# saurabh260918/Graph-Attention-Network-GATv2-

Hardware: AMD Instinct MI355X
Metric: edges/sec (fwd+bwd, 2-layer 8-head GATv2) (higher is better)
Workload: dtype f32; 1 GPU; products-shape synthetic power-law graph, 2450000 nodes / 61900000 edges / 100 feat / 47 classes, 2-layer GATv2 heads [8, 8] outdims [8, 8], fp32; launch=eager, parallelism=single GPU, generator=device (csrc/gat_synth.hip), bit-for-bit synth.py

## Files before the change

graph-attention-network-gatv2-_amd/csrc/gat_dense_kernels.hip:

```cpp
#include "gat_internal.h"

#include <algorithm>
#include <type_traits>

#include <cstdlib>

namespace gat {
namespace {

struct MapIdentity {
    __device__ __forceinline__ int64_t operator()(int64_t idx) const { return idx; }
};
struct MapGradW {
    int32_t HD, F, c_base;
    __device__ __forceinline__ int64_t operator()(int64_t idx) const {
        const int32_t c = c_base + (int32_t)idx / F, f = (int32_t)idx % F;
        return (int64_t)(c % HD) * 2 * F + (c / HD) * F + f;
    }
};
template <class MAP>
__global__ __launch_bounds__(1024) void reduce_slabs_kernel(const float* __restrict__ slabs, int32_t nslabs,
                                                           int64_t width, float* __restrict__ out, MAP map) {
    __shared__ float part[16][64];
    const int q = threadIdx.x & 63, sl = threadIdx.x >> 6;
    const int64_t idx = (int64_t)blockIdx.x * 64 + q;
    float s0 = 0.f, s1 = 0.f, s2 = 0.f, s3 = 0.f;
    if (idx < width) {
        int z = sl;
        for (; z + 48 < nslabs; z += 64) {
            s0 += slabs[(int64_t)z * width + idx];
            s1 += slabs[(int64_t)(z + 16) * width + idx];
            s2 += slabs[(int64_t)(z + 32) * width + idx];
            s3 += slabs[(int64_t)(z + 48) * width + idx];
        }
        for (; z < nslabs; z += 16) s0 += slabs[(int64_t)z * width + idx];
    }
    part[sl][q] = (s0 + s1) + (s2 + s3);
    __syncthreads();
    if (sl == 0 && idx < width) {
        float tot = 0.f;
#pragma unroll
        for (int w = 0; w < 16; ++w) tot += part[w][q];
        out[map(idx)] += tot;
    }
}

__global__ __launch_bounds__(1024) void reduce_batch_kernel(ReduceBatch B) {
    __shared__ float part[16][64];
    if ((int)blockIdx.x >= B.blocks) {
        if (threadIdx.x >= 64) return;
        float lossv = 0.f; int32_t corrv = 0;
        if (B.fin_loss != nullptr) {
            double l = 0.0; int c = 0;
            for (int i = threadIdx.x; i < B.fin_n; i += 64) { l += B.fin_loss[i]; c += B.fin_corr[i]; }
            for (int off = 32; off > 0; off >>= 1) { l += __shfl_down(l, off); c += __shfl_down(c, off); }
            lossv = (float)l; corrv = c;
            if (threadIdx.x == 0) { *B.fin_loss_out = lossv; *B.fin_corr_out = corrv; }
        } else if (threadIdx.x == 0 && B.dst3 != nullptr) {
            lossv = *B.loss; corrv = *B.correct;
        }
        if (threadIdx.x == 0 && B.dst3 != nullptr) {
            const float v0 = lossv, v1 = (float)(corrv & 4095), v2 = (float)(corrv >> 12);
            B.dst3[0] = v0; B.dst3[1] = v1; B.dst3[2] = v2;
            if (B.dst3_host != nullptr) { B.dst3_host[0] = v0; B.dst3_host[1] = v1; B.dst3_host[2] = v2; }
        }
        return;
    }
    int j = 0;
#pragma unroll
    for (int i = 1; i < 8; ++i) if (i < B.n && (int)blockIdx.x >= B.jobs[i].block0) j = i;
    const ReduceJob J = B.jobs[j];
    const int q = threadIdx.x & 63, sl = threadIdx.x >> 6;
    const int64_t idx = (int64_t)((int)blockIdx.x - J.block0) * 64 + q;
    float s0 = 0.f, s1 = 0.f, s2 = 0.f, s3 = 0.f;
    if (idx < J.width) {
        int z = sl;
        for (; z + 48 < J.nslabs; z += 64) {
            s0 += J.slabs[(int64_t)z * J.width + idx];
            s1 += J.slabs[(int64_t)(z + 16) * J.width + idx];
            s2 += J.slabs[(int64_t)(z + 32) * J.width + idx];
            s3 += J.slabs[(int64_t)(z + 48) * J.width + idx];
        }
        for (; z < J.nslabs; z += 16) s0 += J.slabs[(int64_t)z * J.width + idx];
    }
    part[sl][q] = (s0 + s1) + (s2 + s3);
    __syncthreads();
    if (sl == 0 && idx < J.width) {
        float tot = 0.f;
#pragma unroll
        for (int w = 0; w < 16; ++w) tot += part[w][q];
        const int64_t o = J.HD != 0 ? MapGradW{J.HD, J.F, J.c_base}(idx) : idx;
        J.out[o] += tot;
    }
}

template <int DLP>
__global__ __launch_bounds__(256) void head_forward_kernel(HeadArgs A, int32_t NB, int32_t ldz) {
    extern __shared__ float lds[];
    constexpr int DLS = DLP > 0 ? DLP : 1;
    const int C = A.C, DL = A.DL;
    const int wstride = DLP > 0 ? DLP : DL;
    float* s_wo = lds;
    float* s_z = lds + C * wstride;
    __shared__ double s_loss[4];
    __shared__ int32_t s_corr[4];
    for (int i = threadIdx.x; i < C * wstride; i += blockDim.x) {
        const int c = i / wstride, j = i % wstride;
        s_wo[i] = j < DL ? A.Wo[c * DL + j] : 0.f;
    }
    __syncthreads();
    double loss_acc = 0.0;
    int corr_acc = 0;
    const int64_t ntiles = (A.n_rows + NB - 1) / NB;
    const int dq = 256 / C, dr = 256 % C;
    for (int64_t tile = blockIdx.x; tile < ntiles; tile += gridDim.x) {
        const int64_t n0 = tile * NB;
        const int t = threadIdx.x;
        const int64_t n = n0 + t;
        if (t < NB && n < A.n_rows) {
            float* zr = s_z + t * ldz;
            const float* x = A.HL + n * DL;
            float mv = -INFINITY;
            if constexpr (DLP > 0) {
                float xr[DLS];
#pragma unroll
                for (int j = 0; j < DLS; ++j) xr[j] = j < DL ? x[j] : 0.f;
                for (int c = 0; c < C; ++c) {
                    float acc = 0.f;
#pragma unroll
                    for (int j = 0; j < DLS; ++j) acc += s_wo[c * DLS + j] * xr[j];
                    zr[c] = acc;
                    mv = fmaxf(mv, acc);
                }
            } else {
                for (int c = 0; c < C; ++c) {
                    float acc = 0.f;
                    for (int j = 0; j < DL; ++j) acc += s_wo[c * DL + j] * x[j];
                    zr[c] = acc;
                    mv = fmaxf(mv, acc);
                }
            }
            float sum = 0.f;
            for (int c = 0; c < C; ++c) { const float ev = __builtin_amdgcn_exp2f((zr[c] - mv) * 1.4426950408889634f); zr[c] = ev; sum += ev; }
            const double den = (double)sum + 1e-8;
            const double rden = 1.0 / den;
            const int lab = A.labels[n];
            float best = -1.f; int pred = 0; float plab = 0.f;
            for (int c = 0; c < C; ++c) {
                const float yv = (float)((double)zr[c] * rden);
                zr[c] = yv;
                if (c == 0 || yv > best) { best = yv; pred = c; }
                if (c == lab) plab = yv;
            }
            loss_acc += lab >= 0 ? (double)(-logf(fmaxf(plab, 1e-12f))) : 0.0;
            corr_acc += (lab >= 0 && pred == lab) ? 1 : 0;
// ... 126 lines not shown
    const int tid = threadIdx.x;
    const int t2 = tid - 128;
    const int wc = t2 >= 0 ? t2 % C : 0, whalf = t2 >= 0 ? t2 / C : 2;
    float wacc[DL];
#pragma unroll
    for (int d = 0; d < DL; ++d) wacc[d] = 0.f;
    const int64_t ntiles = (A.n_rows + NB - 1) / NB;
    const int dqC = 256 / C, drC = 256 % C;
    for (int64_t tile = blockIdx.x; tile < ntiles; tile += gridDim.x) {
        const int64_t n0 = tile * NB;
        const int rows_here = (int)((A.n_rows - n0 < NB) ? (A.n_rows - n0) : NB);
        __syncthreads();
        {
            const float* yt = A.y + n0 * C;
            int r = tid / C, c = tid % C;
            for (int q = tid; q < rows_here * C; q += 256) {
                const int lab_r = A.labels[n0 + r];
                s_dz[r * ldz + c] = lab_r >= 0 ? yt[q] - (c == lab_r ? 1.0f : 0.0f) : 0.0f;
                r += dqC; c += drC;
                if (c >= C) { c -= C; ++r; }
            }
        }
        for (int q = tid; q < rows_here * DL; q += 256) s_hl[q] = A.HL[n0 * DL + q];
        __syncthreads();
        if (tid < 128) {
            if (tid < rows_here) {
                float acc[DL];
#pragma unroll
                for (int d = 0; d < DL; ++d) acc[d] = 0.f;
                const float* zr = s_dz + tid * ldz;
                for (int c = 0; c < C; ++c) {
                    const float z = zr[c];
#pragma unroll
                    for (int d = 0; d < DL; ++d) acc[d] += s_wo[c * DL + d] * z;
                }
                float* out = A.gh_out + (n0 + tid) * (A.gh_stride ? A.gh_stride : DL);
#pragma unroll
                for (int d = 0; d < DL; ++d) out[d] = acc[d];
            }
        } else if (whalf < 2) {
            const int r0 = whalf * 64, r1 = (r0 + 64 < rows_here) ? r0 + 64 : rows_here;
            for (int r = r0; r < r1; ++r) {
                const float z = s_dz[r * ldz + wc];
#pragma unroll
                for (int d = 0; d < DL; ++d) wacc[d] += z * s_hl[r * DL + d];
            }
        }
    }
    __syncthreads();
    float* s_tmp = s_dz;
    if (whalf < 2) {
#pragma unroll
        for (int d = 0; d < DL; ++d) s_tmp[(whalf * C + wc) * DL + d] = wacc[d];
    }
    __syncthreads();
    for (int i = tid; i < C * DL; i += 256) A.partial[(int64_t)blockIdx.x * C * DL + i] = s_tmp[i] + s_tmp[C * DL + i];
}

template <int DL>
__global__ __launch_bounds__(256) void head_step_kernel(HeadArgs F, HeadBwdArgs A, int32_t ldz) {
    constexpr int NB = 128;
    extern __shared__ float lds[];
    const int C = A.C;
    float* s_wo = lds;
    float* s_dz = s_wo + C * DL;
    float* s_hl = s_dz + NB * ldz;
    __shared__ double s_loss[2];
    __shared__ int32_t s_corr[2];
    for (int i = threadIdx.x; i < C * DL; i += 256) s_wo[i] = A.Wo[i];
    const int tid = threadIdx.x;
    const int t2 = tid - 128;
    const int wc = t2 >= 0 ? t2 % C : 0, whalf = t2 >= 0 ? t2 / C : 2;
    float wacc[DL];
#pragma unroll
    for (int d = 0; d < DL; ++d) wacc[d] = 0.f;
    double loss_acc = 0.0;
    int corr_acc = 0;
    const int64_t ntiles = (A.n_rows + NB - 1) / NB;
    for (int64_t tile = blockIdx.x; tile < ntiles; tile += gridDim.x) {
        const int64_t n0 = tile * NB;
        const int rows_here = (int)((A.n_rows - n0 < NB) ? (A.n_rows - n0) : NB);
        __syncthreads();
        if (tid < rows_here) {
            const int64_t n = n0 + tid;
            float x[DL];
#pragma unroll
            for (int j = 0; j < DL; ++j) { x[j] = A.HL[n * DL + j]; s_hl[tid * DL + j] = x[j]; }
            float* zr = s_dz + tid * ldz;
            float mv = -INFINITY;
            for (int c = 0; c < C; ++c) {
                float acc = 0.f;
#pragma unroll
                for (int j = 0; j < DL; ++j) acc += s_wo[c * DL + j] * x[j];
                zr[c] = acc;
                mv = fmaxf(mv, acc);
            }
            float sum = 0.f;
            for (int c = 0; c < C; ++c) { const float ev = __builtin_amdgcn_exp2f((zr[c] - mv) * 1.4426950408889634f); zr[c] = ev; sum += ev; }
            const double rden = 1.0 / ((double)sum + 1e-8);
            const int lab = A.labels[n];
            float best = -1.f; int pred = 0; float plab = 0.f;
            for (int c = 0; c < C; ++c) {
                const float yv = (float)((double)zr[c] * rden);
                if (c == 0 || yv > best) { best = yv; pred = c; }
                if (c == lab) plab = yv;
                zr[c] = lab >= 0 ? yv - (c == lab ? 1.0f : 0.0f) : 0.0f;
            }
            loss_acc += lab >= 0 ? (double)(-logf(fmaxf(plab, 1e-12f))) : 0.0;
            corr_acc += (lab >= 0 && pred == lab) ? 1 : 0;
        }
        __syncthreads();
        if (tid < 128) {
            if (tid < rows_here) {
                float acc[DL];
#pragma unroll
                for (int d = 0; d < DL; ++d) acc[d] = 0.f;
                const float* zr = s_dz + tid * ldz;
                for (int c = 0; c < C; ++c) {
                    const float z = zr[c];
#pragma unroll
                    for (int d = 0; d < DL; ++d) acc[d] += s_wo[c * DL + d] * z;
                }
                if (A.gh_out != nullptr) {
                    float* out = A.gh_out + (n0 + tid) * (A.gh_stride ? A.gh_stride : DL);
#pragma unroll
                    for (int d = 0; d < DL; ++d) out[d] = acc[d];
                }
            }
        } else if (whalf < 2) {
            const int r0 = whalf * 64, r1 = (r0 + 64 < rows_here) ? r0 + 64 : rows_here;
            for (int r = r0; r < r1; ++r) {
                const float z = s_dz[r * ldz + wc];
#pragma unroll
                for (int d = 0; d < DL; ++d) wacc[d] += z * s_hl[r * DL + d];
            }
        }
    }
    __syncthreads();
    float* s_tmp = s_dz;
    if (whalf < 2) {
#pragma unroll
        for (int d = 0; d < DL; ++d) s_tmp[(whalf * C + wc) * DL + d] = wacc[d];
    }
    for (int off = 32; off > 0; off >>= 1) {
        loss_acc += __shfl_down(loss_acc, off);
        corr_acc += __shfl_down(corr_acc, off);
    }
    if (tid < 128 && (tid & 63) == 0) { s_loss[tid >> 6] = loss_acc; s_corr[tid >> 6] = corr_acc; }
    __syncthreads();
    for (int i = tid; i < C * DL; i += 256) A.partial[(int64_t)blockIdx.x * C * DL + i] = s_tmp[i] + s_tmp[C * DL + i];
    if (tid == 0) {
        F.loss_partial[blockIdx.x] = s_loss[0] + s_loss[1];
        F.correct_partial[blockIdx.x] = s_corr[0] + s_corr[1];
    }
}

__global__ __launch_bounds__(256) void sgd_kernel(float* p, const float* g, float lr, int64_t n) {
    const int64_t i = (int64_t)blockIdx.x * blockDim.x + threadIdx.x;
    if (i < n) p[i] -= lr * g[i];
}
__global__ __launch_bounds__(256) void adam_kernel(float* p, const float* g, float* m, float* v, float lr,
                                                  int64_t n, float b1, float b2, float eps, int32_t t) {
    const int64_t i = (int64_t)blockIdx.x * blockDim.x + threadIdx.x;
    if (i < n) {
        const float gi = g[i];
        const float mi = b1 * m[i] + (1.0f - b1) * gi;
        const float vi = b2 * v[i] + (1.0f - b2) * (gi * gi);
        m[i] = mi; v[i] = vi;
        const float mh = mi / (1.0f - powf(b1, (float)t));
        const float vh = vi / (1.0f - powf(b2, (float)t));
        p[i] -= lr * mh / (sqrtf(vh) + eps);
    }
}
__global__ __launch_bounds__(1024) void sumsq_kernel(const float* __restrict__ g, int64_t n, float* out) {
    __shared__ float part[16];
    float s = 0.f;
    for (int64_t i = threadIdx.x; i < n; i += blockDim.x) s += g[i] * g[i];
    for (int off = 32; off > 0; off >>= 1) s += __shfl_down(s, off);
    if ((threadIdx.x & 63) == 0) part[threadIdx.x >> 6] = s;
    __syncthreads();
    if (threadIdx.x == 0) {
        float t = 0.f;
        for (int w = 0; w < 16; ++w) t += part[w];
        *out = t;
    }
}
__global__ __launch_bounds__(256) void clip_scale_kernel(float* g, int64_t n, const float* sumsq, float thresh) {
    const float norm = sqrtf(*sumsq);
    float scale = 1.0f;
    if (norm > thresh) scale = thresh / (norm + 1e-9f);
    if (!(scale < 1.0f)) return;
    const int64_t i = (int64_t)blockIdx.x * blockDim.x + threadIdx.x;
    if (i < n) g[i] *= scale;
}

template <int V>
__global__ __launch_bounds__(256) void res_backward_kernel(ResBwdArgs A, int32_t LPR, int32_t rpb) {
    __shared__ float red[256 * 4];
    const int HD = A.H * A.D;
    const int t = threadIdx.x;
    const int r_in = t / LPR, cl = t % LPR;
    const float inv_heads = 1.0f / (float)A.H;
    for (int base = 0; base < HD; base += LPR * V) {
        const int c0 = base + cl * V;
        const bool active = r_in < rpb && c0 < HD;
        float sum[V];
        float bv[V];
#pragma unroll
        for (int i = 0; i < V; ++i) { sum[i] = 0.f; bv[i] = (active && A.bias != nullptr) ? A.bias[c0 + i] : 0.f; }
        if (active) {
            for (int64_t row = (int64_t)blockIdx.x * rpb + r_in; row < A.n_rows; row += (int64_t)gridDim.x * rpb) {
                const int64_t o = row * HD + c0;
                float hp[V], gv[V], rv[V];
                if constexpr (V == 4) {
                    const float4 h4 = *reinterpret_cast<const float4*>(A.hpre + o);
                    hp[0] = h4.x; hp[1] = h4.y; hp[2] = h4.z; hp[3] = h4.w;
                    float4 r4 = make_float4(0.f, 0.f, 0.f, 0.f);
                    if (A.res != nullptr) r4 = *reinterpret_cast<const float4*>(A.res + o);
                    rv[0] = r4.x; rv[1] = r4.y; rv[2] = r4.z; rv[3] = r4.w;
                    if (A.gh == nullptr) {
                        const float4 g4 = *reinterpret_cast<const float4*>(A.g + o);
                        gv[0] = g4.x; gv[1] = g4.y; gv[2] = g4.z; gv[3] = g4.w;
                    }
                } else {
                    hp[0] = A.hpre[o];
                    rv[0] = A.res != nullptr ? A.res[o] : 0.f;
                    if (A.gh == nullptr) gv[0] = A.g[o];
                }
                float G[V], ag[V];
#pragma unroll
                for (int i = 0; i < V; ++i) {
                    const float d = hp[i] > 0.f ? 1.0f : A.slope;
                    if (A.gh != nullptr) G[i] = A.gh[row * A.gh_stride + (c0 + i) % A.D] * d * inv_heads;
                    else G[i] = A.g_raw ? gv[i] * d : gv[i];
                    ag[i] = hp[i] - (rv[i] + bv[i]);
                    sum[i] += G[i];
                }
                if constexpr (V == 4) {
                    *reinterpret_cast<float4*>(A.G + o) = make_float4(G[0], G[1], G[2], G[3]);
                    *reinterpret_cast<float4*>(A.agg + o) = make_float4(ag[0], ag[1], ag[2], ag[3]);
                } else {
                    A.G[o] = G[0];
                    A.agg[o] = ag[0];
                }
            }
        }
        if (A.partial != nullptr) {
#pragma unroll
            for (int i = 0; i < V; ++i) red[t * V + i] = sum[i];
            __syncthreads();
            if (r_in == 0 && c0 < HD) {
#pragma unroll
                for (int i = 0; i < V; ++i) {
                    float tot = 0.f;
                    for (int r = 0; r < rpb; ++r) tot += red[(r * LPR + cl) * V + i];
                    A.partial[(int64_t)blockIdx.x * HD + c0 + i] = tot;
                }
            }
            __syncthreads();
        }
    }
}

__device__ __forceinline__ float row_lanes_sum(float x, int LPR) {
    for (int off = LPR >> 1; off > 0; off >>= 1) x += __shfl_xor(x, off);
    return x;
}
template <int V>
__device__ __forceinline__ void load_channels(const float* __restrict__ p, float (&x)[V]) {
    if constexpr (V == 4) {
        const float4 t = *reinterpret_cast<const float4*>(p);
        x[0] = t.x; x[1] = t.y; x[2] = t.z; x[3] = t.w;
    } else {
        x[0] = p[0];
    }
}
template <int V, bool ONE>
__global__ __launch_bounds__(256) void norm_backward_kernel(NormBwdArgs A, int32_t LPR, int32_t rpb) {
    __shared__ float red[256 * 4];
    const ResBwdArgs& R = A.r;
    const int HD = R.H * R.D;
    const int t = threadIdx.x;
    const int r_in = t / LPR, cl = t % LPR;
    const int span = LPR * V;
    const int walk = ONE ? 1 : HD;
    const float inv_heads = 1.0f / (float)R.H, inv_hd = 1.0f / (float)HD;
    auto channels = [&](int64_t row, int c, float mu, float rstd, float (&u)[V], float (&xh)[V], float (&dv)[V], float (&dxh)[V]) {
        load_channels<V>(R.hpre + row * HD + c, u);
        float go[V];
        if (R.gh == nullptr) load_channels<V>(R.g + row * HD + c, go);
#pragma unroll
        for (int i = 0; i < V; ++i) {
            const float gm = A.gamma[c + i];
            xh[i] = (u[i] - mu) * rstd;
            const float v = gm * xh[i] + A.beta[c + i];
            if (R.gh != nullptr) go[i] = R.gh[row * R.gh_stride + (c + i) % R.D] * inv_heads;
            dv[i] = go[i] * (v > 0.f ? 1.0f : R.slope);
            dxh[i] = dv[i] * gm;
        }
    };
    for (int ob = 0; ob < HD; ob += span) {
        const int c0 = ob + cl * V;
        const bool own = c0 < HD;
        float sG[V], sg[V], sb[V], bv[V];
#pragma unroll
        for (int i = 0; i < V; ++i) { sG[i] = 0.f; sg[i] = 0.f; sb[i] = 0.f; bv[i] = (own && R.bias != nullptr) ? R.bias[c0 + i] : 0.f; }
// ... 69 lines not shown
        flush(sg, A.part_gamma);
        flush(sb, A.part_beta);
        flush(sG, R.partial);
    }
}

}

static void res_backward_shape(int32_t HD, int* V, int* LPR, int* rpb) {
    *V = HD % 4 == 0 ? 4 : 1;
    const int groups = HD / *V;
    *LPR = groups < 256 ? groups : 256;
    *rpb = 256 / *LPR;
}
int res_backward_blocks(int64_t n_rows, int32_t HD) {
    int V, LPR, rpb;
    res_backward_shape(HD, &V, &LPR, &rpb);
    const void* fn = V == 4 ? (const void*)res_backward_kernel<4> : (const void*)res_backward_kernel<1>;
    const int64_t want = std::max<int64_t>(1, (n_rows + rpb - 1) / rpb);
    return (int)std::min({want, resident_blocks(fn, 0), (int64_t)kResPartialRows});
}
int launch_res_backward(const ResBwdArgs& a, hipStream_t s) {
    if (a.n_rows <= 0) return 0;
    if (a.blocks < 1 || a.blocks > kResPartialRows) return fail(GAT_E_INVALID, "res_backward: blocks must come from res_backward_blocks()");
    if (a.gh == nullptr && a.g == nullptr) return fail(GAT_E_INVALID, "res_backward: no output gradient");
    int V, LPR, rpb;
    res_backward_shape(a.H * a.D, &V, &LPR, &rpb);
    if (V == 4) hipLaunchKernelGGL(res_backward_kernel<4>, dim3((unsigned)a.blocks), dim3(256), 0, s, a, LPR, rpb);
    else hipLaunchKernelGGL(res_backward_kernel<1>, dim3((unsigned)a.blocks), dim3(256), 0, s, a, LPR, rpb);
    GAT_HIP(hipGetLastError());
    return 0;
}
static void norm_backward_shape(int32_t HD, int* V, int* LPR, int* rpb, bool* one) {
    *V = HD % 4 == 0 ? 4 : 1;
    const int groups = HD / *V;
    int l = 1;
    while (l < groups && l < 64) l <<= 1;
    *LPR = l;
    *rpb = 256 / l;
    *one = groups <= l;
}
static const void* norm_backward_fn(int V, bool one) {
    if (V == 4) return one ? (const void*)norm_backward_kernel<4, true> : (const void*)norm_backward_kernel<4, false>;
    return one ? (const void*)norm_backward_kernel<1, true> : (const void*)norm_backward_kernel<1, false>;
}
int norm_backward_blocks(int64_t n_rows, int32_t HD) {
    int V, LPR, rpb;
    bool one;
    norm_backward_shape(HD, &V, &LPR, &rpb, &one);
    const int64_t want = std::max<int64_t>(1, (n_rows + rpb - 1) / rpb);
    return (int)std::min({want, resident_blocks(norm_backward_fn(V, one), 0), (int64_t)kResPartialRows});
}
int launch_norm_backward(const NormBwdArgs& a, hipStream_t s) {
    if (a.r.n_rows <= 0) return 0;
    if (a.r.blocks < 1 || a.r.blocks > kResPartialRows) return fail(GAT_E_INVALID, "norm_backward: blocks must come from norm_backward_blocks()");
    if (a.r.gh == nullptr && a.r.g == nullptr) return fail(GAT_E_INVALID, "norm_backward: no output gradient");
    if (a.gamma == nullptr || a.beta == nullptr || a.r.G == nullptr || a.r.H < 1 || a.r.D < 1) return fail(GAT_E_INVALID, "norm_backward: null argument");
    int V, LPR, rpb;
    bool one;
    norm_backward_shape(a.r.H * a.r.D, &V, &LPR, &rpb, &one);
    NormBwdArgs arg = a;
    void* args[] = {&arg, &LPR, &rpb};
    GAT_HIP(hipLaunchKernel(norm_backward_fn(V, one), dim3((unsigned)a.r.blocks), dim3(256), args, 0, s));
    return 0;
}
static thread_local ReduceBatch t_batch;
static thread_local bool t_batch_on = false;
void reduce_batch_begin() { t_batch = ReduceBatch{}; t_batch_on = true; }
void reduce_batch_abort() { t_batch_on = false; }
void reduce_batch_pack(const float* loss, const int32_t* correct, float* dst3, float* dst3_host) {
    t_batch.loss = loss; t_batch.correct = correct; t_batch.dst3 = dst3; t_batch.dst3_host = dst3_host;
}
bool reduce_batch_finalize(const double* lp, const int32_t* cp, int32_t nb, float* loss_out, int32_t* correct_out) {
    if (!t_batch_on || t_batch.fin_loss != nullptr) return false;
    t_batch.fin_loss = lp; t_batch.fin_corr = cp; t_batch.fin_n = nb; t_batch.fin_loss_out = loss_out; t_batch.fin_corr_out = correct_out;
    return true;
}
static bool reduce_batch_push(const float* slabs, int32_t nslabs, int64_t width, float* out, int32_t HD, int32_t F, int32_t c_base) {
    if (!t_batch_on || t_batch.n >= 8 || width <= 0) return false;
    ReduceJob& j = t_batch.jobs[t_batch.n++];
    j = ReduceJob{slabs, out, width, nslabs, HD, F, c_base, t_batch.blocks};
    t_batch.blocks += (int32_t)((width + 63) / 64);
    return true;
}
int reduce_batch_flush(hipStream_t s) {
    if (!t_batch_on) return 0;
    t_batch_on = false;
    const int extra = (t_batch.dst3 != nullptr || t_batch.fin_loss != nullptr) ? 1 : 0;
    if (t_batch.blocks + extra == 0) return 0;
    hipLaunchKernelGGL(reduce_batch_kernel, dim3((unsigned)(t_batch.blocks + extra)), dim3(1024), 0, s, t_batch);
    GAT_HIP(hipGetLastError());
    return 0;
}

int launch_reduce_gradw(const float* slabs, int32_t ksplit, int32_t HD, int32_t F, int32_t c_base, int32_t M,
                        float* gradW, hipStream_t s) {
    const int64_t width = (int64_t)M * F;
    if (reduce_batch_push(slabs, ksplit, width, gradW, HD, F, c_base)) return 0;
    hipLaunchKernelGGL((reduce_slabs_kernel<MapGradW>), dim3((unsigned)((width + 63) / 64)), dim3(1024), 0, s, slabs,
                       ksplit, width, gradW, MapGradW{HD, F, c_base});
    GAT_HIP(hipGetLastError());
    return 0;
}

int launch_reduce_partials_add(const float* partial, int32_t nblocks, int64_t width, float* out, hipStream_t s) {
    if (width <= 0) return 0;
    if (reduce_batch_push(partial, nblocks, width, out, 0, 0, 0)) return 0;
    hipLaunchKernelGGL((reduce_slabs_kernel<MapIdentity>), dim3((unsigned)((width + 63) / 64)), dim3(1024), 0, s,
                       partial, nblocks, width, out, MapIdentity{});
    GAT_HIP(hipGetLastError());
    return 0;
}

static int head_tile(int32_t C, int32_t DL, int32_t extra_per_row, int32_t* NB, int32_t* ldz) {
    const int l = (C % 2 == 0) ? C + 1 : C;
    int64_t budget = 60 * 1024 / 4 - (int64_t)C * DL;
    int nb = 256;
    while (nb >= 32 && (int64_t)nb * (l + extra_per_row) > budget) nb >>= 1;
    if (nb < 32) return fail(GAT_E_UNSUPPORTED, "output head: num_classes*D_last too large for the LDS tile");
    *NB = nb; *ldz = l;
    return 0;
}
int head_blocks(int64_t n_rows) {
    static const int per = [] { const char* e = choice_env("GAT_HEAD_NODES"); const int v = e ? atoi(e) : 0; return v == 256 ? 256 : 128; }();
    const int64_t b = (n_rows + per - 1) / per;
    return (int)(b < 1 ? 1 : (b > 2048 ? 2048 : b));
}
int launch_head_forward(const HeadArgs& a, hipStream_t s) {
    int32_t NB, ldz;
    const int dlp = a.DL <= 8 ? 8 : (a.DL <= 16 ? 16 : (a.DL <= 32 ? 32 : (a.DL <= 64 ? 64 : 0)));
    GAT_TRY(head_tile(a.C, dlp ? dlp : a.DL, 0, &NB, &ldz));
    int blocks = head_blocks(a.n_rows);
    const size_t lds = ((size_t)a.C * (dlp ? dlp : a.DL) + (size_t)NB * ldz) * sizeof(float);
    {
        const void* fn = dlp == 8 ? (const void*)head_forward_kernel<8> : dlp == 16 ? (const void*)head_forward_kernel<16>
                       : dlp == 32 ? (const void*)head_forward_kernel<32> : dlp == 64 ? (const void*)head_forward_kernel<64>
                                                                                      : (const void*)head_forward_kernel<0>;
        const int64_t res = resident_blocks(fn, lds);
        if (res < blocks) blocks = (int)res;
    }
    switch (dlp) {
        case 8: hipLaunchKernelGGL(head_forward_kernel<8>, dim3(blocks), dim3(256), lds, s, a, NB, ldz); break;
        case 16: hipLaunchKernelGGL(head_forward_kernel<16>, dim3(blocks), dim3(256), lds, s, a, NB, ldz); break;
        case 32: hipLaunchKernelGGL(head_forward_kernel<32>, dim3(blocks), dim3(256), lds, s, a, NB, ldz); break;
        case 64: hipLaunchKernelGGL(head_forward_kernel<64>, dim3(blocks), dim3(256), lds, s, a, NB, ldz); break;
        default: hipLaunchKernelGGL(head_forward_kernel<0>, dim3(blocks), dim3(256), lds, s, a, NB, ldz); break;
    }
    GAT_HIP(hipGetLastError());
    hipLaunchKernelGGL(head_finalize_kernel, dim3(1), dim3(64), 0, s, a.loss_partial, a.correct_partial, blocks,
                       a.loss_out, a.correct_out);
    GAT_HIP(hipGetLastError());
    return 0;
}
bool head_step_supported(const HeadBwdArgs& b) {
    return b.g == nullptr && b.gh_out != nullptr && b.C <= 64 && (b.DL == 4 || b.DL == 8 || b.DL == 16);
}
int launch_head_step(const HeadArgs& f, const HeadBwdArgs& b, hipStream_t s) {
    HeadBwdArgs probe = b;
    if (probe.gh_out == nullptr) probe.gh_out = reinterpret_cast<float*>(1);
    if (!head_step_supported(probe)) return fail(GAT_E_UNSUPPORTED, "head_step: shape outside the fused kernel");
    const int ldz = (b.C % 2 == 0) ? b.C + 1 : b.C;
    const size_t lds = ((size_t)b.C * b.DL + (size_t)128 * (ldz + b.DL)) * sizeof(float);
    int blocks = std::min(head_blocks(b.n_rows), head_bwd_blocks(b.n_rows, b.C, b.DL));
    const void* fn = b.DL == 4 ? (const void*)head_step_kernel<4> : b.DL == 8 ? (const void*)head_step_kernel<8>
                                                                                : (const void*)head_step_kernel<16>;
    const int64_t res = resident_blocks(fn, lds);
    if (res < blocks) blocks = (int)res;
    if (blocks < 1) blocks = 1;
    if (b.DL == 4) hipLaunchKernelGGL(head_step_kernel<4>, dim3(blocks), dim3(256), lds, s, f, b, ldz);
    else if (b.DL == 8) hipLaunchKernelGGL(head_step_kernel<8>, dim3(blocks), dim3(256), lds, s, f, b, ldz);
    else hipLaunchKernelGGL(head_step_kernel<16>, dim3(blocks), dim3(256), lds, s, f, b, ldz);
    GAT_HIP(hipGetLastError());
    if (!reduce_batch_finalize(f.loss_partial, f.correct_partial, blocks, f.loss_out, f.correct_out)) {
        hipLaunchKernelGGL(head_finalize_kernel, dim3(1), dim3(64), 0, s, f.loss_partial, f.correct_partial, blocks,
                           f.loss_out, f.correct_out);
        GAT_HIP(hipGetLastError());
    }
    return launch_reduce_partials_add(b.partial, blocks, (int64_t)b.C * b.DL, b.gradWo, s);
}
int launch_pack_result(const float* loss, const int32_t* correct, float* dst3, hipStream_t s) {
    hipLaunchKernelGGL(pack_result_kernel, dim3(1), dim3(64), 0, s, loss, correct, dst3);
    GAT_HIP(hipGetLastError());
    return 0;
}
int head_bwd_blocks(int64_t n_rows, int32_t C, int32_t DL) {
    (void)C; (void)DL;
    const int64_t b = (n_rows + 127) / 128;
    return (int)(b < 1 ? 1 : (b > 1024 ? 1024 : b));
}
int launch_head_backward(const HeadBwdArgs& a, hipStream_t s) {
    if (a.g == nullptr && a.gh_out != nullptr && a.C <= 64 && (a.DL == 4 || a.DL == 8 || a.DL == 16)) {
        const int ldz = (a.C % 2 == 0) ? a.C + 1 : a.C;
        const size_t lds = ((size_t)a.C * a.DL + (size_t)128 * (ldz + a.DL)) * sizeof(float);
        int blocks = (int)std::min<int64_t>((a.n_rows + 127) / 128, 1024);
        const void* fn = a.DL == 4 ? (const void*)head_backward2_kernel<4> : a.DL == 8 ? (const void*)head_backward2_kernel<8>
                                                                                        : (const void*)head_backward2_kernel<16>;
        const int64_t res = resident_blocks(fn, lds);
        if (res < blocks) blocks = (int)res;
        if (blocks < 1) blocks = 1;
        if (a.DL == 4) hipLaunchKernelGGL(head_backward2_kernel<4>, dim3(blocks), dim3(256), lds, s, a, ldz);
        else if (a.DL == 8) hipLaunchKernelGGL(head_backward2_kernel<8>, dim3(blocks), dim3(256), lds, s, a, ldz);
        else hipLaunchKernelGGL(head_backward2_kernel<16>, dim3(blocks), dim3(256), lds, s, a, ldz);
        GAT_HIP(hipGetLastError());
        return launch_reduce_partials_add(a.partial, blocks, (int64_t)a.C * a.DL, a.gradWo, s);
    }
    int32_t NB, ldz;
    GAT_TRY(head_tile(a.C, a.DL, 2 * a.DL, &NB, &ldz));
    const int per_thread = (a.C * a.DL + 255) / 256;
    if (per_thread > 8) return fail(GAT_E_UNSUPPORTED, "output head: num_classes*D_last > 2048");
    int blocks = head_bwd_blocks(a.n_rows, a.C, a.DL);
    const size_t lds = ((size_t)a.C * a.DL + (size_t)NB * (ldz + 2 * a.DL)) * sizeof(float);
    {
        const int64_t res = resident_blocks((const void*)head_backward_kernel, lds);
        if (res < blocks) blocks = (int)res;
    }
    hipLaunchKernelGGL(head_backward_kernel, dim3(blocks), dim3(256), lds, s, a, NB, ldz, per_thread);
    GAT_HIP(hipGetLastError());
    return launch_reduce_partials_add(a.partial, blocks, (int64_t)a.C * a.DL, a.gradWo, s);
}

__global__ __launch_bounds__(256) void apply_mask_kernel(const int32_t* __restrict__ labels, const uint8_t* __restrict__ mask,
                                                         int32_t* __restrict__ eff, int64_t n) {
    const int64_t stride = (int64_t)gridDim.x * blockDim.x;
    for (int64_t i = (int64_t)blockIdx.x * blockDim.x + threadIdx.x; i < n; i += stride)
        eff[i] = (mask == nullptr || mask[i]) ? labels[i] : ~labels[i];
}
int launch_apply_mask(const int32_t* labels, const uint8_t* mask, int32_t* eff, int64_t n, hipStream_t s) {
    if (n <= 0) return 0;
    hipLaunchKernelGGL(apply_mask_kernel, dim3((unsigned)std::min<int64_t>((n + 255) / 256, 4096)), dim3(256), 0, s, labels, mask, eff, n);
    GAT_HIP(hipGetLastError());
    return 0;
}
__global__ __launch_bounds__(256) void eval_mask_kernel(const float* __restrict__ y, const int32_t* __restrict__ labels,
                                                        const uint8_t* __restrict__ mask, int64_t n, int32_t C,
                                                        double* __restrict__ part_loss, int32_t* __restrict__ part_cnt) {
    __shared__ double s_l[256];
    __shared__ int32_t s_c[256], s_n[256];
    double l = 0.0; int32_t cr = 0, nn = 0;
    for (int64_t i = (int64_t)blockIdx.x * 256 + threadIdx.x; i < n; i += (int64_t)gridDim.x * 256) {
        if (!mask[i]) continue;
        const float* yr = y + i * C;
        const int lab = labels[i];
        float best = -1.f; int pred = 0;
        for (int c = 0; c < C; ++c) if (c == 0 || yr[c] > best) { best = yr[c]; pred = c; }
        l += (double)(-logf(fmaxf(yr[lab], 1e-12f)));
        cr += pred == lab; ++nn;
    }
    s_l[threadIdx.x] = l; s_c[threadIdx.x] = cr; s_n[threadIdx.x] = nn;
    __syncthreads();
    for (int off = 128; off > 0; off >>= 1) {
        if (threadIdx.x < off) { s_l[threadIdx.x] += s_l[threadIdx.x + off]; s_c[threadIdx.x] += s_c[threadIdx.x + off]; s_n[threadIdx.x] += s_n[threadIdx.x + off]; }
        __syncthreads();
    }
    if (threadIdx.x == 0) { part_loss[blockIdx.x] = s_l[0]; part_cnt[2 * blockIdx.x] = s_c[0]; part_cnt[2 * blockIdx.x + 1] = s_n[0]; }
}
int launch_eval_mask(const float* y, const int32_t* labels, const uint8_t* mask, int64_t n, int32_t C, double* part_loss,
                     int32_t* part_cnt, int32_t blocks, hipStream_t s) {
    hipLaunchKernelGGL(eval_mask_kernel, dim3((unsigned)blocks), dim3(256), 0, s, y, labels, mask, n, C, part_loss, part_cnt);
    GAT_HIP(hipGetLastError());
    return 0;
}

__global__ __launch_bounds__(256) void xavier_init_kernel(float* __restrict__ p, int64_t n, uint64_t s0, uint64_t draw0, float lim) {
    const int64_t stride = (int64_t)gridDim.x * blockDim.x;
    for (int64_t i = (int64_t)blockIdx.x * blockDim.x + threadIdx.x; i < n; i += stride) {
        uint64_t z = s0 + (draw0 + (uint64_t)i + 1ull) * 0x9E3779B97F4A7C15ull;
        z = (z ^ (z >> 30)) * 0xBF58476D1CE4E5B9ull;
        z = (z ^ (z >> 27)) * 0x94D049BB133111EBull;
        z ^= z >> 31;
        const float u = ((float)(z >> 40) + 1.0f) * (1.0f / 16777216.0f);
        p[i] = u * 2.0f * lim - lim;
    }
}
int launch_xavier_init(float* p, int64_t n, uint64_t s0, uint64_t draw0, float lim, hipStream_t s) {
    if (n <= 0) return 0;
    int64_t blocks = (n + 255) / 256;
    if (blocks > 4096) blocks = 4096;
    hipLaunchKernelGGL(xavier_init_kernel, dim3((unsigned)blocks), dim3(256), 0, s, p, n, s0, draw0, lim);
    GAT_HIP(hipGetLastError());
    return 0;
}

int launch_sgd(float* p, const float* g, float lr, int64_t n, hipStream_t s) {
    if (n <= 0) return 0;
    hipLaunchKernelGGL(sgd_kernel, dim3((unsigned)((n + 255) / 256)), dim3(256), 0, s, p, g, lr, n);
    GAT_HIP(hipGetLastError());
    return 0;
}
int launch_adam(float* p, const float* g, float* m, float* v, float lr, int64_t n, float b1, float b2, float eps,
                int32_t t, hipStream_t s) {
    if (n <= 0) return 0;
    hipLaunchKernelGGL(adam_kernel, dim3((unsigned)((n + 255) / 256)), dim3(256), 0, s, p, g, m, v, lr, n, b1, b2,
                       eps, t);
    GAT_HIP(hipGetLastError());
    return 0;
}
int launch_clip(float* g, int64_t n, float thresh, float* scratch, hipStream_t s) {
    if (n <= 0) return 0;
    hipLaunchKernelGGL(sumsq_kernel, dim3(1), dim3(1024), 0, s, g, n, scratch);
    GAT_HIP(hipGetLastError());
    hipLaunchKernelGGL(clip_scale_kernel, dim3((unsigned)((n + 255) / 256)), dim3(256), 0, s, g, n, scratch, thresh);
    GAT_HIP(hipGetLastError());
    return 0;
}

namespace {

template <int MODE>
__device__ __forceinline__ void loss_entry(float z, float t, float& y, float& l, float& dz, int& ok) {
    if constexpr (MODE == GAT_LOSS_BCE) {
        const float e = __builtin_amdgcn_exp2f(-fabsf(z) * 1.4426950408889634f);
        const float r = __builtin_amdgcn_rcpf(1.0f + e);
        y = z >= 0.f ? r : e * r;
// ... 420 lines not shown
```

Before: 3.026 billion edges/s.

## Add per-lane fused head step kernel with wave-local LDS gradW accumulation

Adds a new fused output-head forward+backward kernel in which each lane processes a full row: it computes the logits against an LDS-staged transposed Wo, then the softmax, loss and gradient to h. The weight-gradient outer product is accumulated per wave through LDS slabs using wave-level barriers instead of block barriers, and the next tile's inputs are prefetched. The kernel is templated over the class-group count and selected by default for large row counts when pointers are aligned. It trades more registers per lane and extra template instantiations for fewer block-wide syncs and less shuffling.

Result: no change. 3.048 billion edges/s (median of 6 runs) (+0.7%).

```diff
diff --git a/graph-attention-network-gatv2-_amd/csrc/gat_dense_kernels.hip b/graph-attention-network-gatv2-_amd/csrc/gat_dense_kernels.hip
--- a/graph-attention-network-gatv2-_amd/csrc/gat_dense_kernels.hip
+++ b/graph-attention-network-gatv2-_amd/csrc/gat_dense_kernels.hip
@@ -1,6 +1,7 @@
 #include "gat_internal.h"
 
 #include <algorithm>
+#include <utility>
 #include <type_traits>
 
 #include <cstdlib>
@@ -433,6 +434,229 @@
     if (tid == 0) {
         F.loss_partial[blockIdx.x] = s_loss[0] + s_loss[1];
         F.correct_partial[blockIdx.x] = s_corr[0] + s_corr[1];
+    }
+}
+
+__device__ __forceinline__ void wave_lds_sync() {
+    __builtin_amdgcn_fence(__ATOMIC_RELEASE, "wavefront");
+    __builtin_amdgcn_wave_barrier();
+    __builtin_amdgcn_fence(__ATOMIC_ACQUIRE, "wavefront");
+}
+typedef float lanes_f2 __attribute__((ext_vector_type(2)));
+template <int DL, bool FULL, int ZN>
+__device__ __forceinline__ void lanes_logits(const float* wt, int C, int g, const float (&x)[DL], float (&z)[ZN], float& mv) {
+#pragma clang fp contract(off)
+    lanes_f2 a01 = {0.f, 0.f}, a23 = {0.f, 0.f};
+#pragma unroll
+    for (int j = 0; j < DL; ++j) {
+        const float4 w4 = *reinterpret_cast<const float4*>(wt + j * ZN + 4 * g);
+        const lanes_f2 xx = {x[j], x[j]};
+        const lanes_f2 p01 = lanes_f2{w4.x, w4.y} * xx, p23 = lanes_f2{w4.z, w4.w} * xx;
+        a01 = a01 + p01;
+        a23 = a23 + p23;
+    }
+    z[4 * g] = a01.x; z[4 * g + 1] = a01.y; z[4 * g + 2] = a23.x; z[4 * g + 3] = a23.y;
+#pragma unroll
+    for (int k = 0; k < 4; ++k) {
+        const int c = 4 * g + k;
+        if (FULL || c < C) mv = fmaxf(mv, z[c]);
+        else z[c] = 0.f;
+    }
+}
+template <bool FULL, int ZN>
+__device__ __forceinline__ void lanes_exp(int C, int g, float mv, float (&z)[ZN], float& sum) {
+    if (FULL) {
+#pragma unroll
+        for (int k = 0; k < 4; k += 2) {
+            const int c = 4 * g + k;
+            const lanes_f2 t = (lanes_f2{z[c], z[c + 1]} - lanes_f2{mv, mv}) * lanes_f2{1.4426950408889634f, 1.4426950408889634f};
+            const float e0 = __builtin_amdgcn_exp2f(t.x), e1 = __builtin_amdgcn_exp2f(t.y);
+            z[c] = e0; z[c + 1] = e1;
+            sum += e0;
+            sum += e1;
+        }
+        return;
+    }
+#pragma unroll
+    for (int k = 0; k < 4; ++k) {
+        const int c = 4 * g + k;
+        if (c < C) { const float ev = __builtin_amdgcn_exp2f((z[c] - mv) * 1.4426950408889634f); z[c] = ev; sum += ev; }
+    }
+}
+template <bool FULL, int ZN>
+__device__ __forceinline__ void lanes_dz(int C, int g, double rden, int lab, float (&z)[ZN], float& best, int& pred, float& plab) {
+#pragma unroll
+    for (int k = 0; k < 4; ++k) {
+        const int c = 4 * g + k;
+        if (FULL || c < C) {
+            const float yv = (float)((double)z[c] * rden);
+            if (c == 0 || yv > best) { best = yv; pred = c; }
+            if (c == lab) plab = yv;
+            z[c] = yv - (c == lab ? 1.0f : 0.0f);
+        }
+    }
+}
+template <int DL, bool FULL, int ZN>
+__device__ __forceinline__ void lanes_gh(const float* __restrict__ Wo, int C, int g, const float (&z)[ZN], float (&acc)[DL]) {
+#pragma unroll
+    for (int k = 0; k < 4; ++k) {
+        const int c = 4 * g + k;
+        if (FULL || c < C) {
+#pragma unroll
+            for (int d = 0; d < DL; ++d) acc[d] = __builtin_fmaf(Wo[c * DL + d], z[c], acc[d]);
+        }
+    }
+}
+template <int DL, int NG>
+__global__ __launch_bounds__(256) void head_step_lanes_kernel(HeadArgs F, HeadBwdArgs A, const float* __restrict__ Wo, int32_t ldz) {
+    constexpr int ng = NG;
+    constexpr int NB = 256, V = DL / 4;
+    extern __shared__ float lds[];
+    __shared__ double s_loss[4];
+    __shared__ int32_t s_corr[4];
+    const int C = A.C;
+    const int tid = threadIdx.x, lane = tid & 63, wave = tid >> 6;
+    constexpr int R = 32;
+    float* s_wt = lds;
+    float* w_dz = lds + DL * 4 * NG + wave * R * (ldz + DL);
+    float* w_hl = w_dz + R * ldz;
+    const int ns = 64 / ng, nps = (R + ns - 1) / ns;
+    const int pg = lane % ng, ps = lane / ng;
+    const float4* __restrict__ HL4 = reinterpret_cast<const float4*>(A.HL);
+    const int32_t* __restrict__ labels = A.labels;
+    const int gstride = A.gh_stride ? A.gh_stride : DL;
+    float wacc[4][DL];
+#pragma unroll
+    for (int k = 0; k < 4; ++k)
+#pragma unroll
+        for (int d = 0; d < DL; ++d) wacc[k][d] = 0.f;
+    double loss_acc = 0.0;
+    int corr_acc = 0;
+    const int64_t ntiles = (A.n_rows + NB - 1) / NB;
+    float4 xn[V];
+    int labn = -1;
+    {
+        const int64_t n = (int64_t)blockIdx.x * NB + tid;
+        if (blockIdx.x < ntiles && n < A.n_rows) {
+#pragma unroll
+            for (int v = 0; v < V; ++v) xn[v] = HL4[n * V + v];
+            labn = labels[n];
+        }
+    }
+    for (int i = tid; i < DL * 4 * NG; i += 256) {
+        const int j = i / (4 * NG), c = i % (4 * NG);
+        s_wt[i] = c < C ? Wo[c * DL + j] : 0.f;
+    }
+    __syncthreads();
+    for (int64_t tile = blockIdx.x; tile < ntiles; tile += gridDim.x) {
+        const int64_t n = tile * NB + tid;
+        const int64_t left = A.n_rows - (tile * NB + wave * 64);
+        const int wrows = left >= 64 ? 64 : (left > 0 ? (int)left : 0);
+        float x[DL];
+#pragma unroll
+        for (int v = 0; v < V; ++v) { x[4 * v] = xn[v].x; x[4 * v + 1] = xn[v].y; x[4 * v + 2] = xn[v].z; x[4 * v + 3] = xn[v].w; }
+        const int lab = labn;
+        {
+            const int64_t nn = n + (int64_t)gridDim.x * NB;
+            if (tile + gridDim.x < ntiles && nn < A.n_rows) {
+#pragma unroll
+                for (int v = 0; v < V; ++v) xn[v] = HL4[nn * V + v];
+                labn = labels[nn];
+            }
+        }
+        if (wrows == 0) continue;
+        float z[4 * NG];
+        if (lane < wrows) {
+            float mv = -INFINITY;
+#pragma unroll
+            for (int g = 0; g < NG - 1; ++g) lanes_logits<DL, true>(s_wt, C, g, x, z, mv);
+            lanes_logits<DL, false>(s_wt, C, NG - 1, x, z, mv);
+            float sum = 0.f;
+#pragma unroll
+            for (int g = 0; g < NG - 1; ++g) lanes_exp<true>(C, g, mv, z, sum);
+            lanes_exp<false>(C, NG - 1, mv, z, sum);
+            const double rden = lab >= 0 ? 1.0 / ((double)sum + 1e-8) : 0.0;
+            float best = -1.f; int pred = 0; float plab = 0.f;
+#pragma unroll
+            for (int g = 0; g < NG - 1; ++g) lanes_dz<true>(C, g, rden, lab, z, best, pred, plab);
+            lanes_dz<false>(C, NG - 1, rden, lab, z, best, pred, plab);
+            loss_acc += lab >= 0 ? (double)(-logf(fmaxf(plab, 1e-12f))) : 0.0;
+            corr_acc += (lab >= 0 && pred == lab) ? 1 : 0;
+            if (A.gh_out != nullptr) {
+                int wg = 0;
+                asm volatile("" : "+s"(wg));
+                float acc[DL];
+#pragma unroll
+                for (int d = 0; d < DL; ++d) acc[d] = 0.f;
+#pragma unroll
+                for (int g = 0; g < NG - 1; ++g) lanes_gh<DL, true>(Wo + wg, C, g, z, acc);
+                lanes_gh<DL, false>(Wo + wg, C, NG - 1, z, acc);
+                float4* out = reinterpret_cast<float4*>(A.gh_out + n * gstride);
+#pragma unroll
+                for (int v = 0; v < V; ++v) out[v] = make_float4(acc[4 * v], acc[4 * v + 1], acc[4 * v + 2], acc[4 * v + 3]);
+            }
+        }
+        for (int half = 0; half < 2; ++half) {
+            const int hrows = wrows - half * R;
+            if (hrows <= 0) break;
+            if ((lane >> 5) == half && lane < wrows) {
+                const int row = lane & (R - 1);
+#pragma unroll
+                for (int g = 0; g < NG; ++g)
+                    *reinterpret_cast<float4*>(w_dz + row * ldz + 4 * g) = make_float4(z[4 * g], z[4 * g + 1], z[4 * g + 2], z[4 * g + 3]);
+#pragma unroll
+                for (int v = 0; v < V; ++v) *reinterpret_cast<float4*>(w_hl + row * DL + 4 * v) = make_float4(x[4 * v], x[4 * v + 1], x[4 * v + 2], x[4 * v + 3]);
+            }
+            wave_lds_sync();
+            const int r0 = ps * nps;
+            int r1 = r0 + nps;
+            if (r1 > hrows) r1 = hrows;
+            if (r1 > R) r1 = R;
+            for (int r = r0; r < r1; ++r) {
+                const float4 z4 = *reinterpret_cast<const float4*>(w_dz + r * ldz + 4 * pg);
+                const float zk[4] = {z4.x, z4.y, z4.z, z4.w};
+                float h[DL];
+#pragma unroll
+                for (int v = 0; v < V; ++v) {
+                    const float4 h4 = *reinterpret_cast<const float4*>(w_hl + r * DL + 4 * v);
+                    h[4 * v] = h4.x; h[4 * v + 1] = h4.y; h[4 * v + 2] = h4.z; h[4 * v + 3] = h4.w;
+                }
+#pragma unroll
+                for (int k = 0; k < 4; ++k)
+#pragma unroll
+                    for (int d = 0; d < DL; ++d) wacc[k][d] += zk[k] * h[d];
+            }
+            wave_lds_sync();
+        }
+    }
+    for (int off = 32; off > 0; off >>= 1) {
+        loss_acc += __shfl_down(loss_acc, off);
+        corr_acc += __shfl_down(corr_acc, off);
+    }
+    if (lane == 0) { s_loss[wave] = loss_acc; s_corr[wave] = corr_acc; }
+    float* s_all = lds;
+    for (int k = 0; k < 4; ++k) {
+        __syncthreads();
+#pragma unroll
+        for (int kk = 0; kk < 4; ++kk)
+            if (kk == k) {
+#pragma unroll
+                for (int d = 0; d < DL; ++d) s_all[tid * DL + d] = wacc[kk][d];
+            }
+        __syncthreads();
+        for (int o = tid; o < ng * DL; o += 256) {
+            const int g = o / DL, d = o % DL, c = 4 * g + k;
+            if (c < C) {
+                float tot = 0.f;
+                for (int w = 0; w < 4; ++w)
+                    for (int s = 0; s < ns; ++s) tot += s_all[(w * 64 + s * ng + g) * DL + d];
+                A.partial[(int64_t)blockIdx.x * C * DL + c * DL + d] = tot;
+            }
+        }
+    }
+    if (tid == 0) {
+        F.loss_partial[blockIdx.x] = (s_loss[0] + s_loss[1]) + (s_loss[2] + s_loss[3]);
+        F.correct_partial[blockIdx.x] = s_corr[0] + s_corr[1] + s_corr[2] + s_corr[3];
     }
 }
 
@@ -808,6 +1032,11 @@
     GAT_HIP(hipGetLastError());
     return 0;
 }
+template <int DL, int... I>
+static const void* lanes_fn(int ng, std::integer_sequence<int, I...>) {
+    static const void* const table[] = {(const void*)head_step_lanes_kernel<DL, I + 1>...};
+    return table[ng - 1];
+}
 bool head_step_supported(const HeadBwdArgs& b) {
     return b.g == nullptr && b.gh_out != nullptr && b.C <= 64 && (b.DL == 4 || b.DL == 8 || b.DL == 16);
 }
@@ -815,6 +1044,30 @@
     HeadBwdArgs probe = b;
     if (probe.gh_out == nullptr) probe.gh_out = reinterpret_cast<float*>(1);
     if (!head_step_supported(probe)) return fail(GAT_E_UNSUPPORTED, "head_step: shape outside the fused kernel");
+    constexpr int64_t kHeadLanesRows = 65536;
+    static const int form = [] { const char* e = choice_env("GAT_HEAD_STEP"); return e ? atoi(e) : 0; }();
+    const bool aligned = (reinterpret_cast<uintptr_t>(b.HL) & 15) == 0 && (reinterpret_cast<uintptr_t>(b.gh_out) & 15) == 0 && b.gh_stride % 4 == 0;
+    if ((form == 2 || (form != 1 && b.n_rows >= kHeadLanesRows)) && aligned) {
+        const int ng = (b.C + 3) / 4;
+        const int ldz = 4 * (ng | 1);
+        const size_t lds = (size_t)std::max(b.DL * 4 * ng + 128 * (ldz + b.DL), 256 * b.DL) * sizeof(float);
+        const auto all = std::make_integer_sequence<int, 16>();
+        const void* fn = b.DL == 4 ? lanes_fn<4>(ng, all) : b.DL == 8 ? lanes_fn<8>(ng, all) : lanes_fn<16>(ng, all);
+        int blocks = (int)std::min<int64_t>({(b.n_rows + 255) / 256, (int64_t)head_blocks(b.n_rows), (int64_t)head_bwd_blocks(b.n_rows, b.C, b.DL),
+                                             resident_blocks(fn, lds)});
+        if (blocks < 1) blocks = 1;
+        HeadArgs fa = f; HeadBwdArgs ba = b;
+        const float* wo = b.Wo;
+        int32_t ldz_arg = ldz;
+        void* args[] = {&fa, &ba, &wo, &ldz_arg};
+        GAT_HIP(hipLaunchKernel(fn, dim3(blocks), dim3(256), args, lds, s));
+        if (!reduce_batch_finalize(f.loss_partial, f.correct_partial, blocks, f.loss_out, f.correct_out)) {
+            hipLaunchKernelGGL(head_finalize_kernel, dim3(1), dim3(64), 0, s, f.loss_partial, f.correct_partial, blocks,
+                               f.loss_out, f.correct_out);
+            GAT_HIP(hipGetLastError());
+        }
+        return launch_reduce_partials_add(b.partial, blocks, (int64_t)b.C * b.DL, b.gradWo, s);
+    }
     const int ldz = (b.C % 2 == 0) ? b.C + 1 : b.C;
     const size_t lds = ((size_t)b.C * b.DL + (size_t)128 * (ldz + b.DL)) * sizeof(float);
     int blocks = std::min(head_blocks(b.n_rows), head_bwd_blocks(b.n_rows, b.C, b.DL));
```
